# tzeitim/rogtk

Measured on AMD Instinct MI355X. Metric: reads/s UMI score+cluster, 150 bp/12 bp UMI, 1→8 MI355X; % HBM roofline, higher is better.
Workload: dtype u32/f64

## Files before the change

rogtk_amd/csrc/cluster_kernels.hip:

```cpp
#include <hip/hip_ext.h>
#include <hipcub/hipcub.hpp>

#include <algorithm>
#include <cstdlib>
#include <map>
#include <mutex>

#include <atomic>
#include <thread>
#include <chrono>
#include <cstring>

#include "rogtk_internal.h"

namespace rogtk {
namespace {

constexpr int kBlock = 256;
constexpr int kMarkParts = 8;
constexpr int kMarkChunks = 256;
constexpr int kScanWords = 1024;
constexpr int kLocal8Words = 1024;
constexpr int kLocal8Cap = 8192;
constexpr int kLocal8BigCap = 16384;
constexpr int kMaxRounds = 64;
constexpr int kRoundBatch = 4;

enum StatSlot { S_NDISTINCT = 0, S_NCLUSTERS = 1, S_OVERFLOW = 2, S_REDO = 3, S_ROUNDS = 4, S_P0 = 6,
                S_LCAP = 7 };
constexpr int kFlagsOff = 64;
constexpr int kStatsBytes = kFlagsOff + 4 * kMaxRounds;

__device__ __forceinline__ uint64_t rt_word(const uint4 e) { return (uint64_t)e.x | ((uint64_t)e.y << 32); }

__device__ __forceinline__ uint32_t rt_rank(const uint4 e, uint32_t code) {
    return e.z + (uint32_t)__popcll(rt_word(e) & ((1ull << (code & 63)) - 1ull));
}


__global__ __launch_bounds__(kBlock) void k_bitmap_wide(uint8_t* __restrict__ pres, int64_t words,
                                                        uint64_t* __restrict__ out) {
    const int64_t lane_g = (int64_t)blockIdx.x * kBlock + threadIdx.x;
    const int64_t w = lane_g >> 2;
    uint32_t m16 = 0;
    if (w < words) {
        uint4* p = reinterpret_cast<uint4*>(pres) + lane_g;
        const uint4 v = *p;
        const uint32_t x[4] = {v.x, v.y, v.z, v.w};
#pragma unroll
        for (int q = 0; q < 4; ++q) {
            const uint32_t b = x[q] & 0x01010101u;
            m16 |= ((b | (b >> 7) | (b >> 14) | (b >> 21)) & 0xFu) << (4 * q);
        }
        if (v.x | v.y | v.z | v.w) *p = make_uint4(0, 0, 0, 0);
    }
    uint64_t word = (uint64_t)m16 << (16 * (threadIdx.x & 3));
    word |= __shfl_xor(word, 1);
    word |= __shfl_xor(word, 2);
    if ((threadIdx.x & 3) == 0 && w < words) out[w] = word;
}

__global__ void k_bitmap_small(uint8_t* __restrict__ pres, uint64_t nbits, uint64_t* __restrict__ out) {
    if (threadIdx.x != 0 || blockIdx.x != 0) return;
    uint64_t m = 0;
    for (uint64_t b = 0; b < nbits; ++b) {
        if (pres[b]) m |= 1ull << b;
        pres[b] = 0;
    }
    out[0] = m;
}

template <int NT = kBlock>
__device__ __forceinline__ uint32_t block_excl_scan(uint32_t v, uint32_t* s_wave, uint32_t& total) {
    const int lane = threadIdx.x & 63, wave = threadIdx.x >> 6;
    uint32_t incl = v;
#pragma unroll
    for (int off = 1; off < 64; off <<= 1) {
        const uint32_t t = __shfl_up(incl, off);
        if (lane >= off) incl += t;
    }
    if (lane == 63) s_wave[wave] = incl;
    __syncthreads();
    uint32_t before = 0;
    total = 0;
#pragma unroll
    for (int k = 0; k < NT / 64; ++k) {
        const uint32_t s = s_wave[k];
        if (k < wave) before += s;
        total += s;
    }
    __syncthreads();
    return before + incl - v;
}

__global__ __launch_bounds__(kBlock) void k_scan_words(const uint64_t* __restrict__ bitmaps,
                                                       int n_bitmaps, int64_t words,
                                                       const unsigned long long* __restrict__ count_dev,
                                                       uint64_t* __restrict__ G,
                                                       uint32_t* __restrict__ wpref,
                                                       uint32_t* __restrict__ blksum) {
    __shared__ uint32_t s_wave[kBlock / 64];
    int64_t live = words;
    if (count_dev) live = min<int64_t>(words, (int64_t)((*count_dev + 63) / 64));
    const int64_t w0 = (int64_t)blockIdx.x * kScanWords + 4 * threadIdx.x;
    uint32_t c[4];
    uint32_t tsum = 0;
    uint64_t v[4] = {0, 0, 0, 0};
    for (int r = 0; r < n_bitmaps; ++r) {
        const uint64_t* b = bitmaps + (int64_t)r * words;
#pragma unroll
        for (int k = 0; k < 4; ++k)
// ... 962 lines not shown
                        if ((adj[a] >> b) & 1u) mn = root[b] < mn ? root[b] : mn;
                    x[0] = root[a];
                    x[1] = mn;
                    crossed |= CHECK ? x[0] != x[1] : hook_roots(T, f, x, 2, last_x, last_mn);
                }
            } else {
                uint64_t mm = multi;
                while (mm) {
                    const int b = __ffsll((long long)mm) - 1;
                    mm &= mm - 1;
                    const uint64_t below = (1ull << b) - 1ull;
                    int k = 0;
#pragma unroll
                    for (int v = 0; v < 4; ++v)
                        if ((m[v] >> b) & 1ull)
                            x[k++] = root[v] != kNone ? root[v]
                                                      : f[e[v].z + (uint32_t)__popcll(m[v] & below)];
                    if (CHECK) {
                        for (int v = 1; v < k; ++v) crossed |= x[v] != x[0];
                    } else {
                        crossed |= hook_roots(T, f, x, k, last_x, last_mn);
                    }
                }
            }
        }
    }
    const uint64_t crossed_bits = __ballot(crossed);
    if ((threadIdx.x & 63) == 0) {
        if (!CHECK && (u >> 6) < active_words) next[u >> 6] = crossed_bits;
        if (crossed_bits) flags[round] = 1u;
    }
    if (CHECK) return;
    __syncthreads();
    for (int k = threadIdx.x; k < kHookSlots; k += kBlock) {
        const uint32_t x = T.key[k];
        if (x == kNone) continue;
        if (T.val[k] < f[x]) atomicMin(f + x, T.val[k]);
    }
}

__global__ __launch_bounds__(kBlock) void k_hook_g(const uint4* __restrict__ RT, const uint32_t* __restrict__ UR,
                                                   int64_t words, int L, int p0, uint32_t* f,
                                                   unsigned int* __restrict__ flags, int round,
                                                   uint64_t* __restrict__ active, int64_t active_words,
                                                   const unsigned long long* __restrict__ stats) {
    hook_block<false>(blockIdx.x, RT, UR, words, L, p0, f, flags, round, active, active_words, stats);
}

__device__ __forceinline__ int64_t live_distinct(const unsigned long long* stats, int64_t max_distinct) {
    return min<int64_t>((int64_t)stats[S_NDISTINCT], max_distinct);
}

__global__ __launch_bounds__(kBlock) void k_jump(uint32_t* f, const uint64_t* __restrict__ lroot,
                                                 int64_t max_distinct,
                                                 const unsigned long long* __restrict__ stats,
                                                 const unsigned int* __restrict__ flags, int round) {
    if (flags[round] == 0 || stats[S_REDO]) return;
    const int64_t nd = live_distinct(stats, max_distinct);
    const int lane = threadIdx.x & 63;
    const int64_t nwaves = (int64_t)gridDim.x * (kBlock / 64);
    for (int64_t w = ((int64_t)blockIdx.x * kBlock + threadIdx.x) >> 6; w * 64 < nd; w += nwaves) {
        const uint64_t lr = lroot[w];
        const int64_t i = w * 64 + lane;
        if (!((lr >> lane) & 1ull) || i >= nd) continue;
        uint32_t r = f[i];
        if (r == (uint32_t)i) continue;
        for (uint32_t p = f[r]; p != r; p = f[r]) r = p;
        f[i] = r;
    }
}

constexpr int kRootWords = 64;

__device__ __forceinline__ void publish_stats(const unsigned long long* stats, unsigned long long* host,
                                              unsigned long long epoch) {
    for (int k = threadIdx.x; k < kStatsBytes / 8; k += blockDim.x)
        __hip_atomic_store(host + k, stats[k], __ATOMIC_RELAXED, __HIP_MEMORY_SCOPE_SYSTEM);
    __syncthreads();
    if (threadIdx.x == 0) {
        __hip_atomic_store(host + kStatsBytes / 8, epoch, __ATOMIC_RELEASE, __HIP_MEMORY_SCOPE_SYSTEM);
    }
}

__device__ __forceinline__ void roots_block(const int64_t bid, const uint32_t* __restrict__ f,
                                            const uint64_t* __restrict__ lroot, int64_t max_distinct,
                                            int64_t rwords, uint64_t* __restrict__ rbits,
                                            uint32_t* __restrict__ rpref, uint32_t* rblksum,
                                            const unsigned long long* stats) {
    __shared__ uint32_t s_cnt[kRootWords];
    const int64_t nd = live_distinct(stats, max_distinct);
    const int lane = threadIdx.x & 63, wave = threadIdx.x >> 6;
    constexpr int kPerWave = kRootWords / (kBlock / 64);
    const int64_t w0 = bid * kRootWords + wave * kPerWave;
    uint32_t fv[kPerWave];
    uint64_t lr[kPerWave];
#pragma unroll
    for (int k = 0; k < kPerWave; ++k) {
        const int64_t i = (w0 + k) * 64 + lane;
        lr[k] = (w0 + k) * 64 < nd ? lroot[w0 + k] : 0ull;
        fv[k] = i < nd ? f[i] : 0u;
    }
    uint64_t mine = 0;
#pragma unroll
    for (int k = 0; k < kPerWave; ++k) {
        const int64_t i = (w0 + k) * 64 + lane;
        const uint64_t m = __ballot(i < nd && ((lr[k] >> lane) & 1ull) && fv[k] == (uint32_t)i);
        if (lane == k) mine = m;
    }
    if (lane < kPerWave) {
        const int64_t w = w0 + lane;
        if (w < rwords) rbits[w] = mine;
        s_cnt[wave * kPerWave + lane] = (uint32_t)__popcll(mine);
    }
    __syncthreads();
    if (wave == 0) {
        const uint32_t v = lane < kRootWords ? s_cnt[lane] : 0u;
        uint32_t incl = v;
#pragma unroll
        for (int off = 1; off < 64; off <<= 1) {
            const uint32_t t = __shfl_up(incl, off);
            if (lane >= off) incl += t;
        }
        const int64_t w = bid * kRootWords + lane;
        if (lane < kRootWords && w < rwords) rpref[w] = incl - v;
        if (lane == kRootWords - 1) rblksum[bid] = incl;
    }
}

__global__ __launch_bounds__(kBlock) void k_roots_scan(const uint32_t* __restrict__ f,
                                                       const uint64_t* __restrict__ lroot, int64_t max_distinct,
                                                       int64_t rwords, uint64_t* __restrict__ rbits,
                                                       uint32_t* __restrict__ rpref, uint32_t* rblksum,
                                                       const unsigned long long* stats, unsigned long long* host,
                                                       unsigned long long epoch) {
    if (host && blockIdx.x == 0) publish_stats(stats, host, epoch);
    roots_block(blockIdx.x, f, lroot, max_distinct, rwords, rbits, rpref, rblksum, stats);
}

__global__ __launch_bounds__(kBlock) void k_roots_check(const uint32_t* __restrict__ f,
                                                        const uint64_t* __restrict__ lroot, int64_t max_distinct,
                                                        int64_t rwords, uint64_t* __restrict__ rbits,
                                                        uint32_t* __restrict__ rpref, uint32_t* rblksum,
                                                        const unsigned long long* stats, int64_t rblocks,
                                                        const uint4* __restrict__ RT, const uint32_t* __restrict__ UR,
                                                        int64_t words, int L, int p0, unsigned int* flags, int round,
                                                        uint64_t* active, int64_t active_words) {
    if ((int64_t)blockIdx.x < rblocks)
        roots_block(blockIdx.x, f, lroot, max_distinct, rwords, rbits, rpref, rblksum, stats);
    else
        hook_block<true>((int64_t)blockIdx.x - rblocks, RT, UR, words, L, p0, const_cast<uint32_t*>(f), flags,
                                round, active, active_words, stats);
}

__device__ __forceinline__ uint32_t root_label(uint32_t r, const uint64_t* __restrict__ rbits,
                                               const uint32_t* __restrict__ rpref,
                                               const uint32_t* __restrict__ rblkoff) {
    const uint32_t w = r >> 6;
    return rblkoff[w / kRootWords] + rpref[w] + (uint32_t)__popcll(rbits[w] & ((1ull << (r & 63)) - 1ull));
}

__device__ __forceinline__ void put_label(uint64_t c, uint32_t i, uint32_t lab, uint32_t* __restrict__ labelcode,
                                          uint32_t* __restrict__ ilab) {
    if (labelcode) labelcode[c] = lab;
    else ilab[i] = lab;
}

__global__ __launch_bounds__(kBlock) void k_word_label(const uint32_t* __restrict__ f,
                                                       const uint32_t* __restrict__ UR, int64_t words,
                                                       const uint4* __restrict__ RT, int64_t max_distinct,
                                                       const uint64_t* __restrict__ rbits,
                                                       const uint32_t* __restrict__ rpref,
                                                       const uint32_t* __restrict__ rblkoff,
                                                       uint32_t* __restrict__ wlab, uint64_t* __restrict__ wexc,
                                                       uint32_t* __restrict__ labelcode, uint32_t* __restrict__ ilab,
                                                       int exc1_on,
                                                       const uint32_t* __restrict__ rblksum = nullptr,
                                                       int64_t nrb_max = 0, unsigned long long* stats = nullptr,
                                                       const unsigned long long* pstats = nullptr,
                                                       unsigned long long* host = nullptr,
                                                       unsigned long long epoch = 0) {
    extern __shared__ uint32_t s_roff[];
    __shared__ uint32_t s_wave[kBlock / 64];
    if (host && blockIdx.x == 0) publish_stats(pstats, host, epoch);
    if (pstats[S_REDO]) return;
    if (rblksum) {
        const int64_t nd = live_distinct(stats, max_distinct);
        const int64_t nrb = min<int64_t>(nrb_max, (nd + (int64_t)kRootWords * 64 - 1) / ((int64_t)kRootWords * 64));
        uint32_t carry = 0;
        for (int64_t b0 = 0; b0 < nrb; b0 += kBlock) {
            const int64_t b = b0 + threadIdx.x;
            const uint32_t v = b < nrb ? rblksum[b] : 0u;
            uint32_t total;
            const uint32_t ex = block_excl_scan(v, s_wave, total);
            if (b < nrb) s_roff[b] = carry + ex;
            carry += total;
        }
        if (threadIdx.x == 0) {
            s_roff[nrb] = carry;
            if (blockIdx.x == 0) stats[S_NCLUSTERS] = carry;
        }
        __syncthreads();
        rblkoff = s_roff;
    }
    for (int64_t w = (int64_t)blockIdx.x * kBlock + threadIdx.x; w < words; w += (int64_t)gridDim.x * kBlock) {
        const uint32_t ur = UR[w];
        uint32_t root = kNone;
        uint64_t exc = 0;
        uint4 e = make_uint4(0, 0, 0, 0);
        uint64_t m = 0;
        if (ur != kNone) {
            root = f[ur];
        } else {
            e = RT[w];
            m = rt_word(e);
            const int cnt = __popcll(m);
            if (cnt > 0 && (int64_t)e.z + cnt <= max_distinct) {
                uint32_t cand = f[e.z], votes = 1;
                for (int k = 1; k < cnt; ++k) {
                    const uint32_t r = f[e.z + k];
                    if (r == cand) ++votes;
                    else if (votes == 0) {
                        cand = r;
                        votes = 1;
                    } else {
                        --votes;
                    }
                }
                root = cand;
                uint64_t mm = m;
                for (int k = 0; mm; ++k) {
                    const int b = __ffsll((long long)mm) - 1;
                    mm &= mm - 1;
                    if (f[e.z + k] != cand) exc |= 1ull << b;
                }
            }
        }
        uint32_t lab = root != kNone ? root_label(root, rbits, rpref, rblkoff) : kNone;
        if (exc && lab != kNone) {
            const uint64_t rest = exc & (exc - 1);
            if (exc1_on && !rest && lab < (1u << 24)) {
                lab |= 0xC0000000u | ((uint32_t)(__ffsll((long long)exc) - 1) << 24);
            } else if (exc1_on && !(rest & (rest - 1)) && lab < (1u << 17)) {
                lab |= 0xA0000000u | ((uint32_t)(__ffsll((long long)exc) - 1) << 17) |
                       ((uint32_t)(__ffsll((long long)rest) - 1) << 23);
            } else {
                lab = lab < 0x20000000u ? (lab | 0x80000000u) : kNone;
            }
        }
        wlab[w] = lab;
        uint64_t per_code = lab == kNone ? m : exc;
        while (per_code) {
            const int b = __ffsll((long long)per_code) - 1;
            per_code &= per_code - 1;
            const uint32_t i = e.z + (uint32_t)__popcll(m & ((1ull << b) - 1ull));
            if ((int64_t)i >= max_distinct) continue;
            const uint32_t li = root_label(f[i], rbits, rpref, rblkoff);
            put_label((uint64_t)w * 64 + b, i, li, labelcode, ilab);
        }
        wexc[w] = exc;
    }
}

__device__ __forceinline__ uint32_t word_label_of(const uint32_t* __restrict__ wlab,
                                                  const uint64_t* __restrict__ wexc, uint64_t c) {
    return decode_word_label(wlab[c >> 6], wexc, c);
}

template <int MODE, int G>
__global__ __launch_bounds__(kBlock) void k_assign(const uint32_t* __restrict__ codes,
                                                   const uint64_t* __restrict__ regbits, int64_t n,
                                                   const uint32_t* __restrict__ labelcode,
                                                   const uint32_t* __restrict__ flab,
                                                   const uint4* __restrict__ RT, const uint32_t* __restrict__ wlab,
                                                   const uint64_t* __restrict__ wexc, uint32_t* __restrict__ out) {
    constexpr int64_t kTile = 256 * G;
    const int lane = threadIdx.x & 63;
    const int64_t nwaves = (int64_t)gridDim.x * (kBlock / 64);
    for (int64_t tile = (((int64_t)blockIdx.x * kBlock + threadIdx.x) >> 6) * kTile; tile < n;
         tile += nwaves * kTile) {
        uint32_t c[G][4];
        uint32_t reg[G];
#pragma unroll
        for (int g = 0; g < G; ++g) {
            const int64_t row0 = tile + 256 * g + 4 * lane;
            c[g][0] = c[g][1] = c[g][2] = c[g][3] = 0;
            if (row0 + 4 <= n) {
                const u32x4_t v = stream_load(reinterpret_cast<const u32x4_t*>(codes + row0));
                c[g][0] = v.x; c[g][1] = v.y; c[g][2] = v.z; c[g][3] = v.w;
            } else {
                for (int k = 0; k < 4; ++k)
                    if (row0 + k < n) c[g][k] = codes[row0 + k];
            }
            reg[g] = row0 >= n ? 0u : regbits ? (uint32_t)(regbits[row0 >> 6] >> (row0 & 63)) & 0xFu : 0xFu;
        }
        uint32_t id[G][4];
#pragma unroll
        for (int g = 0; g < G; ++g)
#pragma unroll
            for (int k = 0; k < 4; ++k) {
                id[g][k] = 0xFFFFFFFFu;
                if ((reg[g] >> k) & 1u) {
                    const uint32_t wl = wlab ? word_label_of(wlab, wexc, c[g][k]) : kNone;
                    id[g][k] = wl != kNone ? wl
                               : MODE == 0 ? labelcode[c[g][k]]
                               : MODE == 1 ? flab[rt_rank(RT[c[g][k] >> 6], c[g][k])]
                                           : rt_rank(RT[c[g][k] >> 6], c[g][k]);
                }
            }
#pragma unroll
        for (int g = 0; g < G; ++g) {
            const int64_t row0 = tile + 256 * g + 4 * lane;
            if (row0 + 4 <= n) {
                stream_store(u32x4_t{id[g][0], id[g][1], id[g][2], id[g][3]}, reinterpret_cast<u32x4_t*>(out + row0));
            } else {
                for (int k = 0; k < 4; ++k)
                    if (row0 + k < n) out[row0 + k] = id[g][k];
            }
        }
    }
}

template <int MODE>
__global__ __launch_bounds__(kBlock) void k_lookup(const uint64_t* __restrict__ q, int64_t nq, uint64_t nbits,
                                                   const uint32_t* __restrict__ labelcode,
                                                   const uint32_t* __restrict__ flab, const uint4* __restrict__ RT,
                                                   const uint32_t* __restrict__ wlab,
                                                   const uint64_t* __restrict__ wexc, uint32_t* __restrict__ out) {
    for (int64_t i = (int64_t)blockIdx.x * kBlock + threadIdx.x; i < nq; i += (int64_t)gridDim.x * kBlock) {
        const uint64_t c = q[i];
        uint32_t lab = kNone;
        if (c < nbits) {
            const uint4 e = RT[c >> 6];
            if ((rt_word(e) >> (c & 63)) & 1ull) {
                const uint32_t wl = wlab ? word_label_of(wlab, wexc, c) : kNone;
                lab = wl != kNone ? wl : MODE == 0 ? labelcode[c] : flab[rt_rank(e, (uint32_t)c)];
            }
        }
        out[i] = lab;
    }
}

inline int grid_for(int64_t lanes, int64_t cap = 0) {
    int64_t g = (lanes + kBlock - 1) / kBlock;
    if (g < 1) g = 1;
    if (cap && g > cap) g = cap;
    return (int)g;
}

struct WsPtrs {
    unsigned long long* stats;
    unsigned int* flags;
    uint8_t* presence;
    uint64_t* G;
    uint4* RT;
    uint32_t *wpref, *blksum, *blkoff, *D, *f, *UR;
    uint64_t *rbits, *lroot;
    uint32_t *rpref, *rblksum, *rblkoff, *labelcode, *ilab;
    uint64_t* active;
    uint64_t* lb;
};

inline WsPtrs ws_ptrs(const ClusterLayout& cl, uint8_t* ws) {
    WsPtrs p;
    p.stats = (unsigned long long*)(ws + cl.off_stats);
    p.flags = (unsigned int*)(ws + cl.off_stats + kFlagsOff);
    p.presence = ws + cl.off_presence;
    p.G = (uint64_t*)(ws + cl.off_bitmap);
    p.RT = (uint4*)(ws + cl.off_rt);
    p.wpref = (uint32_t*)(ws + cl.off_wpref);
    p.blksum = (uint32_t*)(ws + cl.off_blksum);
    p.blkoff = (uint32_t*)(ws + cl.off_blkoff);
    p.D = (uint32_t*)(ws + cl.off_D);
    p.f = (uint32_t*)(ws + cl.off_f);
    p.UR = (uint32_t*)(ws + cl.off_ur);
    p.rbits = (uint64_t*)(ws + cl.off_rbits);
    p.lroot = (uint64_t*)(ws + cl.off_lroot);
    p.rpref = (uint32_t*)(ws + cl.off_rpref);
    p.rblksum = (uint32_t*)(ws + cl.off_rblksum);
    p.rblkoff = (uint32_t*)(ws + cl.off_rblkoff);
    p.labelcode = cl.label_by_code ? (uint32_t*)(ws + cl.off_labelcode) : nullptr;
    p.ilab = cl.label_by_code ? nullptr : (uint32_t*)(ws + cl.off_ilab);
    p.active = (uint64_t*)(ws + cl.off_active);
    p.lb = (uint64_t*)(ws + cl.off_lb);
    return p;
}

constexpr int64_t kPersistentGrid = 2048;

}

int cluster_layout(int L, int64_t max_distinct, ClusterLayout* o) {
    ROGTK_REQUIRE(L >= 1 && L <= kMaxPackedLen, ROGTK_E_UNSUPPORTED,
                  "cluster: umi_len %d outside 1..%d", L, kMaxPackedLen);
    ROGTK_REQUIRE(max_distinct >= 1 && max_distinct <= 0xFFFFFFFFll, ROGTK_E_INVALID,
                  "cluster: max_distinct %lld outside 1..2^32-1", (long long)max_distinct);
    ClusterLayout c{};
    c.L = L;
    c.nbits = 1ull << (2 * L);
    if ((uint64_t)max_distinct > c.nbits) max_distinct = (int64_t)c.nbits;
    c.max_distinct = max_distinct;
    c.words = (int64_t)((c.nbits + 63) / 64);
    c.blocks = (c.words + kScanWords - 1) / kScanWords;
    c.rwords = (max_distinct + 63) / 64;
    c.rblocks = (c.rwords + kRootWords - 1) / kRootWords;
    c.label_by_code = L <= 13;
    int64_t off = 0;
    auto take = [&](int64_t bytes) {
        const int64_t at = off;
        off += (bytes + 255) / 256 * 256;
        return at;
    };
    c.off_stats = take(kStatsBytes);
    c.off_presence = take((int64_t)(c.nbits < 64 ? 64 : c.nbits));
    c.off_bitmap = take(c.words * 8);
    c.off_rt = take(c.words * 16);
    c.off_wpref = take(c.words * 4);
    c.off_blksum = take(c.blocks * 4);
    c.off_blkoff = take((c.blocks + 1) * 4);
    c.off_D = take(max_distinct * 4);
    c.off_f = take(max_distinct * 4);
    c.off_ur = take(c.words * 4);
    c.off_rbits = take(c.rwords * 8);
    c.off_lroot = take(c.rwords * 8);
    c.off_rpref = take(c.rwords * 4);
    c.off_rblksum = take(c.rblocks * 4);
    c.off_rblkoff = take((c.rblocks + 1) * 4);
    c.off_labelcode = c.label_by_code ? take((int64_t)c.nbits * 4) : off;
    c.off_ilab = c.label_by_code ? off : take(max_distinct * 4);
    const int64_t tasks = L > kLocalPos ? (int64_t)(L - kLocalPos) * (c.words >> 2) : 0;
    c.active_words = (tasks + 63) / 64;
    c.off_active = take(2 * std::max<int64_t>(c.active_words, 1) * 8);
    c.off_lb = take((2 * std::max(c.blocks, c.rblocks) + 1) * 8);
    c.total = off;
    *o = c;
    return ROGTK_OK;
}


__global__ __launch_bounds__(kBlock) void k_mark_xcd(const uint32_t* __restrict__ codes,
                                                      const uint64_t* __restrict__ regbits, int64_t n,
                                                      int two_l, int64_t chunk, uint8_t* __restrict__ pres) {
    const uint32_t part = blockIdx.x % kMarkParts;
    const int64_t c0 = (int64_t)(blockIdx.x / kMarkParts) * chunk;
    const int64_t c1 = c0 + chunk < n ? c0 + chunk : n;
    for (int64_t r = c0 + 4 * (int64_t)threadIdx.x; r < c1; r += 4 * kBlock) {
        uint32_t c[4];
        uint32_t reg = regbits ? (uint32_t)(regbits[r >> 6] >> (r & 63)) & 0xFu : 0xFu;
        if (r + 4 <= n) {
            const u32x4_t v = stream_load(reinterpret_cast<const u32x4_t*>(codes + r));
            c[0] = v.x; c[1] = v.y; c[2] = v.z; c[3] = v.w;
        } else {
            reg &= (1u << (uint32_t)(n - r)) - 1u;
            for (int k = 0; k < 4; ++k) c[k] = r + k < n ? codes[r + k] : 0u;
        }
#pragma unroll
        for (int k = 0; k < 4; ++k)
            if (((reg >> k) & 1u) && (uint32_t)(((uint64_t)c[k] * kMarkParts) >> two_l) == part)
                pres[c[k]] = 1;
    }
}

int launch_cluster_mark(const uint32_t* codes, const uint64_t* regular_bits, int64_t n, int L,
                        uint8_t* presence, hipStream_t s) {
    if (n <= 0) return ROGTK_OK;
    ProfScope prof(K_MARK, s);
    int64_t chunk = (n + kMarkChunks - 1) / kMarkChunks;
    chunk = (chunk + 4 * kBlock - 1) / (4 * kBlock) * (4 * kBlock);
    const int64_t chunks = (n + chunk - 1) / chunk;
    hipLaunchKernelGGL(k_mark_xcd, dim3((unsigned)(chunks * kMarkParts)), dim3(kBlock), 0, s, codes, regular_bits,
                       n, 2 * L, chunk, presence);
    ROGTK_HIP_CHECK(hipGetLastError());
    return ROGTK_OK;
}

int launch_cluster_local_bitmap(const ClusterLayout& cl, uint8_t* ws, uint64_t* out, hipStream_t s) {
    WsPtrs p = ws_ptrs(cl, ws);
    ProfScope prof(K_BITMAP, s);
    if (cl.nbits >= 64) {
        hipLaunchKernelGGL(k_bitmap_wide, dim3(grid_for(cl.words * 4)), dim3(kBlock), 0, s, p.presence,
                           cl.words, out);
    } else {
        hipLaunchKernelGGL(k_bitmap_small, dim3(1), dim3(64), 0, s, p.presence, cl.nbits, out);
    }
    ROGTK_HIP_CHECK(hipGetLastError());
    return ROGTK_OK;
}

namespace {

constexpr int kSpecRounds = 4;
std::atomic<int> g_spec_rounds{kSpecRounds};
std::atomic<bool> g_spec_adaptive{true};
std::atomic<int> g_lb_polls{kLbMaxPolls};

struct ResolveState {
    uint8_t* hstats = nullptr;
    uint8_t* hstats_dev = nullptr;
    uint64_t epoch = 0;
    int launched = 0;
    bool pending = false;
    int rounds = 0;
    int needed = 0;
    bool word_labels = false;
    bool exact = false;
    uint32_t scan_tag = 0;
    int lcc_choice = -1;
    bool checked = false;
    ClusterLayout cl{};
    struct {
        bool on = false;
        const uint32_t* codes;
        const uint64_t* regbits;
        int64_t n;
        uint32_t* cid;
    } deferred;
};
std::mutex g_rs_mu;
std::map<const void*, ResolveState> g_rs;

int wait_published(const ResolveState& st) {
    const volatile unsigned long long* seq = (const volatile unsigned long long*)(st.hstats + kStatsBytes);
    const auto t0 = std::chrono::steady_clock::now();
    while (*seq != st.epoch) {
        std::this_thread::yield();
        ROGTK_REQUIRE(std::chrono::steady_clock::now() - t0 < std::chrono::seconds(120), ROGTK_E_HIP,
                      "cluster: resolve flags not published within 120 s (stream stalled?)");
    }
    std::atomic_thread_fence(std::memory_order_acquire);
    return ROGTK_OK;
}

int enqueue_rounds(const ClusterLayout& cl, const WsPtrs& p, int from, int to, hipStream_t s) {
    const int pg = grid_for(cl.max_distinct, kPersistentGrid);
    const int64_t tasks = (int64_t)(cl.L - kLocalPos) * (cl.words >> 2);
    for (int k = from; k < to; ++k) {
        ROGTK_TIMED_LAUNCH(K_K_HOOK, k_hook_g, dim3(grid_for(tasks)), dim3(kBlock), 0, s, p.RT, p.UR, cl.words, cl.L, kLocalPos,
                           p.f, p.flags, k, p.active, cl.active_words, (const unsigned long long*)p.stats);
        ROGTK_TIMED_LAUNCH(K_K_JUMP, k_jump, dim3(pg), dim3(kBlock), 0, s, p.f, p.lroot, cl.max_distinct, p.stats, p.flags, k);
    }
    ROGTK_HIP_CHECK(hipGetLastError());
    return ROGTK_OK;
}

thread_local hipEvent_t t_resolve_fin = nullptr;

int enqueue_labels(const ClusterLayout& cl, const WsPtrs& p, hipStream_t s,
                   unsigned long long* host_stats = nullptr, int check_round = -1, uint64_t epoch = 0) {
    const bool lds_off = (cl.rblocks + 1) * 4 <= 65536;
    {
        ProfScope prof(K_FLATTEN, s);
        if (check_round >= 0) {
            const int64_t tasks = (int64_t)(cl.L - kLocalPos) * (cl.words >> 2);
            ROGTK_TIMED_LAUNCH(K_K_ROOTS, k_roots_check, dim3((unsigned)(cl.rblocks + grid_for(tasks))), dim3(kBlock), 0, s, p.f,
                               p.lroot, cl.max_distinct, cl.rwords, p.rbits, p.rpref, p.rblksum,
                               (const unsigned long long*)p.stats, cl.rblocks, p.RT, p.UR, cl.words, cl.L, kLocalPos,
                               p.flags, check_round, p.active, cl.active_words);
        } else {
            ROGTK_TIMED_LAUNCH(K_K_ROOTS, k_roots_scan, dim3((unsigned)cl.rblocks), dim3(kBlock), 0, s, p.f, p.lroot,
                               cl.max_distinct, cl.rwords, p.rbits, p.rpref, p.rblksum,
                               (const unsigned long long*)p.stats, host_stats, (unsigned long long)epoch);
        }
        if (!lds_off)
            hipLaunchKernelGGL(k_scan_blocks, dim3(1), dim3(kBlock), 0, s, p.rblksum, cl.rblocks, p.rblkoff, p.stats,
                               (int)S_NCLUSTERS, -1, 0, (int64_t)kRootWords * 64);
        ROGTK_HIP_CHECK(hipGetLastError());
    }
    {
        ProfScope prof(K_LABEL, s);
        static const int exc1_on = [] {
            const char* e = getenv("ROGTK_WORD_EXC1");
            return e && e[0] == '0' ? 0 : 1;
        }();
        if (t_resolve_fin) arm_attached_event(t_resolve_fin);
        ROGTK_TIMED_LAUNCH(K_K_WORD_LABEL, k_word_label, dim3(grid_for(cl.words, kPersistentGrid)), dim3(kBlock),
                           lds_off ? (size_t)(cl.rblocks + 1) * 4 : 0, s, p.f, p.UR, cl.words, p.RT, cl.max_distinct,
                           p.rbits, p.rpref, p.rblkoff, p.wpref, p.G, p.labelcode, p.ilab, exc1_on,
                           lds_off ? p.rblksum : nullptr, (int64_t)cl.rblocks, lds_off ? p.stats : nullptr,
                           (const unsigned long long*)p.stats, check_round >= 0 ? host_stats : nullptr,
                           (unsigned long long)epoch);
        if (t_resolve_fin && attached_event_taken()) t_resolve_fin = nullptr;
        ROGTK_HIP_CHECK(hipGetLastError());
    }
    return ROGTK_OK;
}

int first_zero(const unsigned int* f, int from, int to) {
    for (int k = from; k < to; ++k)
        if (f[k] == 0) return k;
    return -1;
}

}

#ifndef ROGTK_ASSIGN_WGS
#define ROGTK_ASSIGN_WGS 2
#endif
#ifndef ROGTK_ASSIGN_G
#define ROGTK_ASSIGN_G 2
#endif
namespace {
int enqueue_assign(const ClusterLayout& cl, const WsPtrs& p, int labels, const uint32_t* codes,
                   const uint64_t* regular_bits, int64_t n, uint32_t* cluster_id, hipStream_t s);
int finish_locked(const void* ws, ResolveState& st, hipStream_t s, int* redone = nullptr);
}

namespace {
bool fused_scan_enabled() {
    static const bool on = [] {
        const char* e = getenv("ROGTK_FUSED_SCAN");
        return !(e && e[0] == '0');
    }();
    return on;
}

bool lcc_predict_enabled() {
    static const bool on = [] {
        const char* e = getenv("ROGTK_LCC_PREDICT");
        return !(e && e[0] == '0');
    }();
    return on;
}

int enqueue_resolve(const ClusterLayout& cl, const WsPtrs& p, const uint64_t* bitmaps, int n_bitmaps,
                    int max_distance, int spec, unsigned long long* host_stats, uint64_t epoch, hipStream_t s,
                    uint32_t scan_tag, int lcc_choice, bool* checked) {
    *checked = false;
    {
        ProfScope prof(K_SCAN, s);
        if (scan_tag) {
            ROGTK_TIMED_LAUNCH(K_K_SCAN_RT, k_scan_rt, dim3((unsigned)cl.blocks), dim3(kBlock), 0, s, bitmaps, n_bitmaps, cl.words,
                               p.RT, p.lroot, max_distance == 0 ? (int64_t)0 : cl.rwords,
                               p.lb + std::max(cl.blocks, cl.rblocks) + 1, p.lb, scan_tag, p.stats, (int)S_NDISTINCT,
                               max_distance == 0 ? (int)S_NCLUSTERS : -1, local8_enabled() ? cl.L : 0,
                               local8_big_enabled(), g_lb_polls.load());
        } else {
            hipLaunchKernelGGL(k_scan_words, dim3((unsigned)cl.blocks), dim3(kBlock), 0, s, bitmaps, n_bitmaps,
                               cl.words, (const unsigned long long*)nullptr, p.G, p.wpref, p.blksum);
            hipLaunchKernelGGL(k_scan_blocks, dim3(1), dim3(kBlock), 0, s, p.blksum, cl.blocks, p.blkoff, p.stats,
                               (int)S_NDISTINCT, max_distance == 0 ? (int)S_NCLUSTERS : -1, 1, (int64_t)0,
                               local8_enabled() ? cl.L : 0, local8_big_enabled());
            hipLaunchKernelGGL(k_rt, dim3(grid_for(cl.words)), dim3(kBlock), 0, s, p.G, cl.words, p.wpref, p.blkoff,
                               p.RT, p.lroot, max_distance == 0 ? 0 : cl.rwords);
        }
    }
    if (max_distance == 0) {
        const int cgrid = grid_for((int64_t)std::min<uint64_t>(cl.nbits, 1ull << 30), 16384);
        hipLaunchKernelGGL(k_build_d, dim3(cgrid), dim3(kBlock), 0, s, p.RT, cl.nbits, p.D, p.f, p.labelcode, p.ilab,
                           cl.max_distinct, p.stats);
        return hipGetLastError() == hipSuccess ? 0 : -1;
    }
    ProfScope prof(K_UNION, s);
    launch_local_cc(p.RT, cl.words, cl.L, p.f, p.UR, p.lroot, cl.rwords, cl.max_distinct, p.stats, s, lcc_choice);
    if (cl.L <= kLocalPos) {
        if (enqueue_labels(cl, p, s, nullptr)) return -1;
        return hipGetLastError() == hipSuccess ? 0 : -1;
    }
    const bool fuse = host_stats && spec >= 2;
    const int real = fuse ? spec - 1 : spec;
    if (enqueue_rounds(cl, p, 0, real, s)) return -1;
    *checked = fuse;
    if (enqueue_labels(cl, p, s, host_stats, fuse ? real : -1, epoch)) return -1;
    return hipGetLastError() == hipSuccess ? real : -1;
// ... 175 lines not shown
    return enqueue_assign(cl, p, wl, codes, regular_bits, n, cluster_id, s);
}

int cluster_assign_prepare(const ClusterLayout& cl, const uint8_t* ws, const uint32_t* codes,
                           const uint64_t* regular_bits, int64_t n, uint32_t* cluster_id, hipStream_t s,
                           bool deferred, AssignIn* a) {
    a->wlab = nullptr;
    a->wexc = nullptr;
    a->labelcode = nullptr;
    a->out = nullptr;
    if (!deferred)
        if (int rc = cluster_finish(ws, s)) return rc;
    bool wl = false;
    {
        std::lock_guard<std::mutex> lk(g_rs_mu);
        auto it = g_rs.find(ws);
        if (it != g_rs.end()) {
            wl = it->second.word_labels;
            if (deferred && it->second.pending) {
                auto& d = it->second.deferred;
                d.on = true;
                d.codes = codes;
                d.regbits = regular_bits;
                d.n = n;
                d.cid = cluster_id;
            }
        }
    }
    if (!wl || !cl.label_by_code) return ROGTK_OK;
    WsPtrs p = ws_ptrs(cl, const_cast<uint8_t*>(ws));
    a->wlab = p.wpref;
    a->wexc = p.G;
    a->labelcode = p.labelcode;
    a->out = cluster_id;
    return ROGTK_OK;
}

int launch_cluster_lookup(const ClusterLayout& cl, const uint8_t* ws, const uint64_t* q, int64_t nq, uint32_t* lab,
                          hipStream_t s) {
    if (nq <= 0) return ROGTK_OK;
    if (int rc = cluster_finish(ws, s)) return rc;
    WsPtrs p = ws_ptrs(cl, const_cast<uint8_t*>(ws));
    bool wl = false;
    {
        std::lock_guard<std::mutex> lk(g_rs_mu);
        auto it = g_rs.find(ws);
        if (it != g_rs.end()) wl = it->second.word_labels;
    }
    const uint32_t* wlab = wl ? p.wpref : nullptr;
    const uint64_t* wexc = wl ? p.G : nullptr;
    const int g = grid_for(nq, 4096);
    if (cl.label_by_code)
        hipLaunchKernelGGL(k_lookup<0>, dim3(g), dim3(kBlock), 0, s, q, nq, cl.nbits, p.labelcode, p.D, p.RT, wlab,
                           wexc, lab);
    else
        hipLaunchKernelGGL(k_lookup<1>, dim3(g), dim3(kBlock), 0, s, q, nq, cl.nbits, p.labelcode, p.ilab, p.RT, wlab,
                           wexc, lab);
    ROGTK_HIP_CHECK(hipGetLastError());
    return ROGTK_OK;
}

#ifndef ROGTK_ASSIGN_WGS
#define ROGTK_ASSIGN_WGS 2
#endif
#ifndef ROGTK_ASSIGN_G
#define ROGTK_ASSIGN_G 2
#endif
namespace {
int enqueue_assign(const ClusterLayout& cl, const WsPtrs& p, int labels, const uint32_t* codes,
                   const uint64_t* regular_bits, int64_t n, uint32_t* cluster_id, hipStream_t s) {
    if (n <= 0) return ROGTK_OK;
    const uint32_t* wlab = labels == 1 ? p.wpref : nullptr;
    const uint64_t* wexc = labels == 1 ? p.G : nullptr;
    ProfScope prof(K_ASSIGN, s, true);
    static const int64_t cap = [] {
        int dev = 0, cus = 0;
        if (hipGetDevice(&dev) != hipSuccess ||
            hipDeviceGetAttribute(&cus, hipDeviceAttributeMultiprocessorCount, dev) != hipSuccess || cus <= 0)
            cus = 256;
        return (int64_t)ROGTK_ASSIGN_WGS * cus;
    }();
    constexpr int kGroups = ROGTK_ASSIGN_G;
    const int g = grid_for((n + 4 * kGroups - 1) / (4 * kGroups), cap);
    if (labels == 2)
        hipExtLaunchKernelGGL((k_assign<2, kGroups>), dim3(g), dim3(kBlock), 0, s, prof.start(), prof.stop(), 0, codes,
                              regular_bits, n, p.labelcode, p.ilab, p.RT, wlab, wexc, cluster_id);
    else if (cl.label_by_code)
        hipExtLaunchKernelGGL((k_assign<0, kGroups>), dim3(g), dim3(kBlock), 0, s, prof.start(), prof.stop(), 0, codes,
                              regular_bits, n, p.labelcode, p.D, p.RT, wlab, wexc, cluster_id);
    else
        hipExtLaunchKernelGGL((k_assign<1, kGroups>), dim3(g), dim3(kBlock), 0, s, prof.start(), prof.stop(), 0, codes,
                              regular_bits, n, p.labelcode, p.ilab, p.RT, wlab, wexc, cluster_id);
    ROGTK_HIP_CHECK(hipGetLastError());
    return ROGTK_OK;
}
}



namespace {

constexpr int kPartBits = 8;
constexpr int kPartBlock = 512;

__global__ __launch_bounds__(kBlock) void k_mark_keys(const uint32_t* __restrict__ codes,
                                                      const uint64_t* __restrict__ regbits, int64_t n,
                                                      uint32_t* __restrict__ keys) {
    const int64_t i = (int64_t)blockIdx.x * kBlock + threadIdx.x;
    if (i >= n) return;
    const bool reg = (regbits[i >> 6] >> (i & 63)) & 1ull;
    keys[i] = reg ? codes[i] : 0xFFFFFFFFu;
}

__device__ int64_t wg_lower_bound(const uint32_t* __restrict__ a, int64_t n, uint64_t v) {
    int64_t lo = 0, hi = n;
    while (lo < hi) {
        const int64_t step = (hi - lo + kPartBlock - 1) / kPartBlock;
        const int64_t pos = lo + (int64_t)threadIdx.x * step;
        const bool less = pos < hi && (uint64_t)a[pos] < v;
        const int64_t cnt = __syncthreads_count(less);
        const int64_t nlo = cnt ? lo + (cnt - 1) * step + 1 : lo;
        const int64_t nhi = min(hi, lo + cnt * step);
        lo = nlo;
        hi = nhi;
    }
    return lo;
}

__global__ __launch_bounds__(kPartBlock) void k_part_bitmap(const uint32_t* __restrict__ sorted, int64_t n,
                                                            int two_l, uint64_t* __restrict__ bitmap) {
    extern __shared__ uint32_t lbits[];
    const int p = blockIdx.x;
    const int shift = two_l - kPartBits;
    const uint32_t pwords32 = (1u << shift) >> 5;
    for (uint32_t k = threadIdx.x; k < pwords32; k += kPartBlock) lbits[k] = 0;
    __shared__ int64_t range[2];
    const int64_t r0 = wg_lower_bound(sorted, n, (uint64_t)p << shift);
    const int64_t r1 = p + 1 == (1 << kPartBits) ? n : wg_lower_bound(sorted, n, (uint64_t)(p + 1) << shift);
    if (threadIdx.x == 0) {
        range[0] = r0;
        range[1] = r1;
    }
    __syncthreads();
    const uint32_t mask = (1u << shift) - 1u;
    constexpr int kUnroll = 8;
    const int64_t rend = range[1];
    for (int64_t i0 = range[0] + threadIdx.x; i0 < rend; i0 += (int64_t)kPartBlock * kUnroll) {
        uint32_t key[kUnroll];
#pragma unroll
        for (int u = 0; u < kUnroll; ++u) {
            const int64_t i = i0 + (int64_t)u * kPartBlock;
            key[u] = i < rend ? __builtin_nontemporal_load(sorted + i) : 0xFFFFFFFFu;
        }
#pragma unroll
        for (int u = 0; u < kUnroll; ++u) {
            if ((uint64_t)key[u] >> two_l) continue;
            const uint32_t c = key[u] & mask;
            atomicOr(&lbits[c >> 5], 1u << (c & 31));
        }
    }
    __syncthreads();
    uint64_t* out = bitmap + ((uint64_t)p << shift >> 6);
    for (uint32_t k = threadIdx.x; k < pwords32 / 2; k += kPartBlock)
        out[k] = (uint64_t)lbits[2 * k] | ((uint64_t)lbits[2 * k + 1] << 32);
}

#ifndef ROGTK_SLICE_BLOCK
#define ROGTK_SLICE_BLOCK 1024
#endif
constexpr int kSliceBlock = ROGTK_SLICE_BLOCK;
constexpr int kSliceChunks = 8;
#ifndef ROGTK_SLICE_LOG2
#define ROGTK_SLICE_LOG2 20
#endif
constexpr int kSliceLog2 = ROGTK_SLICE_LOG2;
// ... 333 lines not shown
```

rogtk_amd/csrc/rogtk_internal.h:

```cpp
#pragma once

#include <hip/hip_runtime.h>

#include <algorithm>
#include <cstddef>
#include <cstdint>
#include <functional>
#include <vector>

#include "../../include/rogtk_hip.h"

namespace rogtk {

void set_error(const char* fmt, ...) __attribute__((format(printf, 1, 2)));
int require_device();

#define ROGTK_HIP_CHECK(expr)                                                                    \
    do {                                                                                         \
        hipError_t e_ = (expr);                                                                  \
        if (e_ != hipSuccess) {                                                                  \
            ::rogtk::set_error("%s failed: %s (%s:%d)", #expr, hipGetErrorString(e_), __FILE__, \
                               __LINE__);                                                        \
            return ROGTK_E_HIP;                                                                  \
        }                                                                                        \
// ... 121 lines not shown
    if ((wl >> 29) & 1u)
        return b != ((wl >> 17) & 63u) && b != ((wl >> 23) & 63u) ? (wl & 0x1FFFFu) : 0xFFFFFFFFu;
    return ((wexc[c >> 6] >> b) & 1ull) ? 0xFFFFFFFFu : (wl & 0x1FFFFFFFu);
}

#ifndef ROGTK_NT_SCORE_STORE
#define ROGTK_NT_SCORE_STORE 1
#endif
template <class V>
__device__ __forceinline__ void score_store(V v, V* p) {
#if ROGTK_NT_SCORE_STORE
    stream_store(v, p);
#else
    *p = v;
#endif
}

struct PackedParams {
    double sh[kMaxPackedLen + 1];
    double di[kMaxPackedLen + 1];
    double ling[kMaxPackedLen + 1];
    double frac[kMaxPackedLen + 1];
    int L;
    int ham_mode;
    uint32_t tcode, cmplo, always_mismatch, max_distance;
};

struct ScoreOut {
    double* sh;
    double* ling;
    double* homo;
    double* di;
    uint32_t* longest;
    double* dust;
    double* comb;
};

inline ScoreOut to_score_out(const rogtk_umi_scores* s) {
    if (!s) return ScoreOut{nullptr, nullptr, nullptr, nullptr, nullptr, nullptr, nullptr};
    return ScoreOut{s->shannon_entropy,      s->linguistic_complexity, s->homopolymer_fraction,
                    s->dinucleotide_entropy, s->longest_homopolymer_run, s->dust_score,
                    s->combined_score};
}
inline bool any_score(const ScoreOut& o) {
    return o.sh || o.ling || o.homo || o.di || o.longest || o.dust || o.comb;
}

void encode_target(const uint8_t* target, int64_t target_len, int L, uint32_t max_distance,
                   PackedParams* p);
int build_packed_params(int L, PackedParams* p);

struct AssignIn {
    const uint32_t* wlab;
    const uint64_t* wexc;
    const uint32_t* labelcode;
    uint32_t* out;
};

int launch_stage(const void* offsets, int offset_width, const uint8_t* values,
                 const uint8_t* validity, int64_t validity_offset, int64_t n, int L,
                 uint32_t* codes, uint64_t* regular_bits, int64_t* irregular_rows,
                 unsigned long long* n_irregular, hipStream_t s);
int launch_score_packed(const uint32_t* codes, const uint64_t* regular_bits, int64_t n,
                        const PackedParams& p, const ScoreOut& o, uint32_t* hd, uint64_t* hw, hipStream_t s,
                        const AssignIn* asg = nullptr);
int launch_score_rows(const void* offsets, int offset_width, const uint8_t* values,
                      const int64_t* rows, const int64_t* n_rows_dev, int64_t max_rows,
                      const double* lut, int64_t lut_max, const ScoreOut& o,
                      const uint8_t* target_dev, int64_t target_len, int ham, uint32_t max_distance,
                      uint32_t* hd, uint64_t* hw, hipStream_t s);

struct ClusterLayout {
    int L;
    int64_t max_distinct;
    uint64_t nbits;
    int64_t words;
    int64_t blocks;
    int64_t rwords;
    int64_t rblocks;
    bool label_by_code;
    int64_t off_stats, off_presence, off_bitmap, off_rt, off_wpref, off_blksum, off_blkoff, off_D, off_f, off_ur,
        off_rbits, off_lroot, off_rpref, off_rblksum, off_rblkoff, off_labelcode, off_ilab, off_active,
        active_words, off_lb, total;
};
int cluster_layout(int L, int64_t max_distinct, ClusterLayout* out);

struct DevBuf {
    void* p = nullptr;
    size_t cap = 0;
    std::vector<void*> retired;
    ~DevBuf() {
        if (p) hipFree(p);
        for (void* q : retired) hipFree(q);
    }
    int ensure(size_t bytes) {
        if (bytes <= cap && p) return ROGTK_OK;
        size_t grow = 0;
        if (p) {
            retired.push_back(p);
            p = nullptr;
            grow = cap + cap / 2;
            cap = 0;
        }
        size_t want = std::max<size_t>(std::max(bytes, grow), 256);
        want = (want + 255) / 256 * 256;
        ROGTK_HIP_CHECK(hipMalloc(&p, want));
        cap = want;
        return ROGTK_OK;
    }
    void reclaim() {
        for (void* q : retired) hipFree(q);
        retired.clear();
    }
    template <class T>
    T* as() const { return reinterpret_cast<T*>(p); }
};


int launch_cluster_mark(const uint32_t* codes, const uint64_t* regular_bits, int64_t n, int L,
                        uint8_t* presence, hipStream_t s);
int launch_cluster_local_bitmap(const ClusterLayout& cl, uint8_t* ws, uint64_t* bitmap_out,
                                hipStream_t s);
int cluster_mark_bitmap_temp(int64_t n, int L, int64_t* bytes);
int launch_cluster_mark_bitmap(const uint32_t* codes, const uint64_t* regular_bits, int64_t n, int L,
                               uint64_t* bitmap, void* temp, int64_t temp_bytes, hipStream_t s);
int launch_cluster_mark_phase(const uint32_t* codes, const uint64_t* regular_bits, int64_t n, int L,
                              uint64_t* bitmap, void* temp, int64_t temp_bytes, int phase, hipStream_t s);
int cluster_assign_prepare(const ClusterLayout& cl, const uint8_t* ws, const uint32_t* codes,
                           const uint64_t* regular_bits, int64_t n, uint32_t* cluster_id, hipStream_t s,
                           bool deferred, AssignIn* a);
int launch_cluster_resolve(const ClusterLayout& cl, uint8_t* ws, const uint64_t* bitmaps,
                           int n_bitmaps, int max_distance, hipStream_t s);
int cluster_finish(const void* ws, hipStream_t s, int* redone = nullptr);
void cluster_release(const void* ws);
int cluster_rounds(const void* ws, hipStream_t s, int* rounds);
int cluster_set_spec_rounds(int n);
int cluster_set_lookback_polls(int n);
int cluster_set_mark_method(int m);
int launch_cluster_assign(const ClusterLayout& cl, const uint8_t* ws, const uint32_t* codes,
                          const uint64_t* regular_bits, int64_t n, uint32_t* cluster_id,
                          hipStream_t s, bool deferred = false);

int irregular_cluster(const void* offsets, int offset_width, const uint8_t* values,
                      const int64_t* rows, int64_t n_rows, int64_t max_len, const int64_t* stats_dev,
                      uint32_t* cluster_id, int64_t* n_irregular_clusters, hipStream_t s);

using CodeLookup = std::function<int(const uint64_t* q, int64_t nq, uint32_t* lab, hipStream_t s)>;
int irregular_merge(const void* offsets, int offset_width, const uint8_t* values, const int64_t* rows,
                    int64_t n_rows, int64_t max_len, int L, int64_t n_reg, const CodeLookup* lookup,
                    uint32_t* relabel, int64_t relabel_n, uint32_t* cluster_id, int64_t* n_clusters, hipStream_t s);
int sorted_code_lookup(const uint64_t* G, int64_t ng, const uint32_t* labels, const uint64_t* q, int64_t nq,
                       uint32_t* lab, hipStream_t s);
int launch_cluster_lookup(const ClusterLayout& cl, const uint8_t* ws, const uint64_t* q, int64_t nq, uint32_t* lab,
                          hipStream_t s);

int masked_records_range(const uint64_t* D, int64_t nd, int p0, int np, uint64_t* mk, uint32_t* pos, uint64_t* code,
                         hipStream_t s);

int cc_labels(int64_t nv, const uint32_t* edges, int64_t m, uint32_t* labels, int64_t* n_clusters, hipStream_t s);

struct SortedCodes;
struct DevCol;
using ExtraCodeBytes = std::function<int(int64_t m, size_t* bytes)>;
int sorted_distinct_codes(const DevCol& col, int L, bool want_counts, const ExtraCodeBytes* extra, uint32_t* cluster_id,
                          SortedCodes* out, hipStream_t s, const uint32_t* groups = nullptr);

// ... 60 lines not shown
```

Baseline: 38.38 billion.

## Fast-path dominant cluster label in assign via sampled root and LDS bitmap

Samples 256 words in the roots kernel to find a dominant cluster root and stores it in the stats slot. The word-label kernel then writes a per-word bitmap of codes belonging to that root, and the assign kernel loads this bitmap into LDS. Codes found in it take the dominant label directly, skipping the word-label and label-table lookups. This adds sampling work, an extra bitmap write, and LDS use per block that grows with the number of words, which is why it is enabled only for L up to 12.

```diff
diff --git a/rogtk_amd/csrc/cluster_kernels.hip b/rogtk_amd/csrc/cluster_kernels.hip
--- a/rogtk_amd/csrc/cluster_kernels.hip
+++ b/rogtk_amd/csrc/cluster_kernels.hip
@@ -26,7 +26,7 @@
 constexpr int kMaxRounds = 64;
 constexpr int kRoundBatch = 4;
 
-enum StatSlot { S_NDISTINCT = 0, S_NCLUSTERS = 1, S_OVERFLOW = 2, S_REDO = 3, S_ROUNDS = 4, S_P0 = 6,
+enum StatSlot { S_NDISTINCT = 0, S_NCLUSTERS = 1, S_OVERFLOW = 2, S_REDO = 3, S_ROUNDS = 4, S_DOM = 5, S_P0 = 6,
                 S_LCAP = 7 };
 constexpr int kFlagsOff = 64;
 constexpr int kStatsBytes = kFlagsOff + 4 * kMaxRounds;
@@ -1155,6 +1155,47 @@
     }
 }
 
+constexpr int kDomSample = kBlock;
+constexpr int kDomHeader = 2;
+constexpr uint64_t kDomNoLabel = ~0ull;
+constexpr int kDomMaxL = 12;
+
+__device__ __forceinline__ void pick_dominant(const uint32_t* __restrict__ f, const uint32_t* __restrict__ UR,
+                                              const uint4* __restrict__ RT, int64_t words, int64_t max_distinct,
+                                              unsigned long long* dom) {
+    __shared__ uint32_t s_samp[kDomSample];
+    __shared__ unsigned long long s_best[kBlock / 64];
+    const int64_t ns = min<int64_t>(kDomSample, words);
+    const int64_t w = (int64_t)threadIdx.x * (words / ns);
+    uint32_t r = kNone;
+    if ((int64_t)threadIdx.x < ns) {
+        uint32_t i = UR[w];
+        if (i == kNone) {
+            const uint4 e = RT[w];
+            if (rt_word(e)) i = e.z;
+        }
+        if ((int64_t)i < max_distinct) r = f[i];
+    }
+    s_samp[threadIdx.x] = r;
+    __syncthreads();
+    uint32_t cnt = 0;
+    if (r != kNone)
+        for (int k = 0; k < kDomSample; ++k) cnt += s_samp[k] == r;
+    unsigned long long key = r != kNone ? ((unsigned long long)cnt << 32) | (0xFFFFFFFFu - r) : 0ull;
+#pragma unroll
+    for (int off = 32; off; off >>= 1) {
+        const unsigned long long o = __shfl_xor(key, off);
+        key = o > key ? o : key;
+    }
+    if ((threadIdx.x & 63) == 0) s_best[threadIdx.x >> 6] = key;
+    __syncthreads();
+    if (threadIdx.x == 0) {
+        for (int k = 1; k < kBlock / 64; ++k) key = s_best[k] > key ? s_best[k] : key;
+        const bool any = (int64_t)(key >> 32) * 4 >= ns && key != 0;
+        *dom = any ? (unsigned long long)(0xFFFFFFFFu - (uint32_t)key) + 1ull : 0ull;
+    }
+}
+
 __device__ __forceinline__ void roots_block(const int64_t bid, const uint32_t* __restrict__ f,
                                             const uint64_t* __restrict__ lroot, int64_t max_distinct,
                                             int64_t rwords, uint64_t* __restrict__ rbits,
@@ -1205,8 +1246,12 @@
                                                        int64_t rwords, uint64_t* __restrict__ rbits,
                                                        uint32_t* __restrict__ rpref, uint32_t* rblksum,
                                                        const unsigned long long* stats, unsigned long long* host,
-                                                       unsigned long long epoch) {
+                                                       unsigned long long epoch, int64_t rblocks,
+                                                       const uint4* __restrict__ RT, const uint32_t* __restrict__ UR,
+                                                       int64_t words) {
     if (host && blockIdx.x == 0) publish_stats(stats, host, epoch);
+    if ((int64_t)blockIdx.x == (rblocks > 1 ? 1 : 0))
+        pick_dominant(f, UR, RT, words, max_distinct, const_cast<unsigned long long*>(stats) + S_DOM);
     roots_block(blockIdx.x, f, lroot, max_distinct, rwords, rbits, rpref, rblksum, stats);
 }
 
@@ -1218,9 +1263,11 @@
                                                         const uint4* __restrict__ RT, const uint32_t* __restrict__ UR,
                                                         int64_t words, int L, int p0, unsigned int* flags, int round,
                                                         uint64_t* active, int64_t active_words) {
-    if ((int64_t)blockIdx.x < rblocks)
+    if ((int64_t)blockIdx.x < rblocks) {
+        if ((int64_t)blockIdx.x == (rblocks > 1 ? 1 : 0))
+            pick_dominant(f, UR, RT, words, max_distinct, const_cast<unsigned long long*>(stats) + S_DOM);
         roots_block(blockIdx.x, f, lroot, max_distinct, rwords, rbits, rpref, rblksum, stats);
-    else
+    } else
         hook_block<true>((int64_t)blockIdx.x - rblocks, RT, UR, words, L, p0, const_cast<uint32_t*>(f), flags,
                                 round, active, active_words, stats);
 }
@@ -1251,7 +1298,8 @@
                                                        int64_t nrb_max = 0, unsigned long long* stats = nullptr,
                                                        const unsigned long long* pstats = nullptr,
                                                        unsigned long long* host = nullptr,
-                                                       unsigned long long epoch = 0) {
+                                                       unsigned long long epoch = 0,
+                                                       uint64_t* __restrict__ wdom = nullptr) {
     extern __shared__ uint32_t s_roff[];
     __shared__ uint32_t s_wave[kBlock / 64];
     if (host && blockIdx.x == 0) publish_stats(pstats, host, epoch);
@@ -1275,6 +1323,9 @@
         __syncthreads();
         rblkoff = s_roff;
     }
+    const uint32_t dom = wdom ? (uint32_t)pstats[S_DOM] - 1u : kNone;
+    if (wdom && blockIdx.x == 0 && threadIdx.x == 0)
+        wdom[0] = dom != kNone ? (uint64_t)root_label(dom, rbits, rpref, rblkoff) : kDomNoLabel;
     for (int64_t w = (int64_t)blockIdx.x * kBlock + threadIdx.x; w < words; w += (int64_t)gridDim.x * kBlock) {
         const uint32_t ur = UR[w];
         uint32_t root = kNone;
@@ -1321,6 +1372,10 @@
             }
         }
         wlab[w] = lab;
+        if (wdom) {
+            const uint64_t b = __ballot(lab != kNone && root == dom && !exc);
+            if ((threadIdx.x & 63) == 0) wdom[kDomHeader + (w >> 6)] = b;
+        }
         uint64_t per_code = lab == kNone ? m : exc;
         while (per_code) {
             const int b = __ffsll((long long)per_code) - 1;
@@ -1339,13 +1394,31 @@
     return decode_word_label(wlab[c >> 6], wexc, c);
 }
 
-template <int MODE, int G>
+template <int MODE, int G, bool DOM = false>
 __global__ __launch_bounds__(kBlock) void k_assign(const uint32_t* __restrict__ codes,
                                                    const uint64_t* __restrict__ regbits, int64_t n,
                                                    const uint32_t* __restrict__ labelcode,
                                                    const uint32_t* __restrict__ flab,
                                                    const uint4* __restrict__ RT, const uint32_t* __restrict__ wlab,
-                                                   const uint64_t* __restrict__ wexc, uint32_t* __restrict__ out) {
+                                                   const uint64_t* __restrict__ wexc, uint32_t* __restrict__ out,
+                                                   const uint64_t* __restrict__ wdom, int dom_words) {
+    extern __shared__ __attribute__((aligned(16))) uint32_t s_dom[];
+    uint32_t dom_label = 0;
+    bool dom_on = false;
+    if (DOM) {
+        const uint64_t h = wdom[0];
+        dom_on = h != kDomNoLabel;
+        dom_label = (uint32_t)h;
+        if (dom_on) {
+            if (dom_words >= 2) {
+                const uint4* src = reinterpret_cast<const uint4*>(wdom + kDomHeader);
+                for (int i = threadIdx.x; i < dom_words / 2; i += kBlock) reinterpret_cast<uint4*>(s_dom)[i] = src[i];
+            } else if (threadIdx.x < 2) {
+                s_dom[threadIdx.x] = reinterpret_cast<const uint32_t*>(wdom + kDomHeader)[threadIdx.x];
+            }
+            __syncthreads();
+        }
+    }
     constexpr int64_t kTile = 256 * G;
     const int lane = threadIdx.x & 63;
     const int64_t nwaves = (int64_t)gridDim.x * (kBlock / 64);
@@ -1373,6 +1446,10 @@
             for (int k = 0; k < 4; ++k) {
                 id[g][k] = 0xFFFFFFFFu;
                 if ((reg[g] >> k) & 1u) {
+                    if (DOM && dom_on && ((s_dom[c[g][k] >> 11] >> ((c[g][k] >> 6) & 31u)) & 1u)) {
+                        id[g][k] = dom_label;
+                        continue;
+                    }
                     const uint32_t wl = wlab ? word_label_of(wlab, wexc, c[g][k]) : kNone;
                     id[g][k] = wl != kNone ? wl
                                : MODE == 0 ? labelcode[c[g][k]]
@@ -1431,6 +1508,7 @@
     uint32_t *rpref, *rblksum, *rblkoff, *labelcode, *ilab;
     uint64_t* active;
     uint64_t* lb;
+    uint64_t* wdom;
 };
 
 inline WsPtrs ws_ptrs(const ClusterLayout& cl, uint8_t* ws) {
@@ -1455,6 +1533,7 @@
     p.ilab = cl.label_by_code ? nullptr : (uint32_t*)(ws + cl.off_ilab);
     p.active = (uint64_t*)(ws + cl.off_active);
     p.lb = (uint64_t*)(ws + cl.off_lb);
+    p.wdom = cl.dom_words ? (uint64_t*)(ws + cl.off_wdom) : nullptr;
     return p;
 }
 
@@ -1504,6 +1583,8 @@
     c.active_words = (tasks + 63) / 64;
     c.off_active = take(2 * std::max<int64_t>(c.active_words, 1) * 8);
     c.off_lb = take((2 * std::max(c.blocks, c.rblocks) + 1) * 8);
+    c.dom_words = L <= kDomMaxL ? (c.words + 63) / 64 : 0;
+    c.off_wdom = take(c.dom_words ? (kDomHeader + c.dom_words + 1) * 8 : 0);
     c.total = off;
     *o = c;
     return ROGTK_OK;
@@ -1631,7 +1712,8 @@
         } else {
             ROGTK_TIMED_LAUNCH(K_K_ROOTS, k_roots_scan, dim3((unsigned)cl.rblocks), dim3(kBlock), 0, s, p.f, p.lroot,
                                cl.max_distinct, cl.rwords, p.rbits, p.rpref, p.rblksum,
-                               (const unsigned long long*)p.stats, host_stats, (unsigned long long)epoch);
+                               (const unsigned long long*)p.stats, host_stats, (unsigned long long)epoch, cl.rblocks,
+                               p.RT, p.UR, cl.words);
         }
         if (!lds_off)
             hipLaunchKernelGGL(k_scan_blocks, dim3(1), dim3(kBlock), 0, s, p.rblksum, cl.rblocks, p.rblkoff, p.stats,
@@ -1650,7 +1732,7 @@
                            p.rbits, p.rpref, p.rblkoff, p.wpref, p.G, p.labelcode, p.ilab, exc1_on,
                            lds_off ? p.rblksum : nullptr, (int64_t)cl.rblocks, lds_off ? p.stats : nullptr,
                            (const unsigned long long*)p.stats, check_round >= 0 ? host_stats : nullptr,
-                           (unsigned long long)epoch);
+                           (unsigned long long)epoch, p.wdom);
         if (t_resolve_fin && attached_event_taken()) t_resolve_fin = nullptr;
         ROGTK_HIP_CHECK(hipGetLastError());
     }
@@ -1992,15 +2074,27 @@
     }();
     constexpr int kGroups = ROGTK_ASSIGN_G;
     const int g = grid_for((n + 4 * kGroups - 1) / (4 * kGroups), cap);
-    if (labels == 2)
+    static const bool dom_on = [] {
+        const char* e = getenv("ROGTK_ASSIGN_DOM");
+        return !(e && e[0] == '0');
+    }();
+    if (labels == 1 && cl.label_by_code && p.wdom && dom_on) {
+        const int dw = (int)cl.dom_words;
+        hipExtLaunchKernelGGL((k_assign<0, kGroups, true>), dim3(g), dim3(kBlock), (size_t)(dw + (dw & 1)) * 8, s,
+                              prof.start(), prof.stop(), 0, codes, regular_bits, n, p.labelcode, p.D, p.RT, wlab, wexc,
+                              cluster_id, (const uint64_t*)p.wdom, dw);
+    } else if (labels == 2)
         hipExtLaunchKernelGGL((k_assign<2, kGroups>), dim3(g), dim3(kBlock), 0, s, prof.start(), prof.stop(), 0, codes,
-                              regular_bits, n, p.labelcode, p.ilab, p.RT, wlab, wexc, cluster_id);
+                              regular_bits, n, p.labelcode, p.ilab, p.RT, wlab, wexc, cluster_id,
+                              (const uint64_t*)nullptr, 0);
     else if (cl.label_by_code)
         hipExtLaunchKernelGGL((k_assign<0, kGroups>), dim3(g), dim3(kBlock), 0, s, prof.start(), prof.stop(), 0, codes,
-                              regular_bits, n, p.labelcode, p.D, p.RT, wlab, wexc, cluster_id);
+                              regular_bits, n, p.labelcode, p.D, p.RT, wlab, wexc, cluster_id,
+                              (const uint64_t*)nullptr, 0);
     else
         hipExtLaunchKernelGGL((k_assign<1, kGroups>), dim3(g), dim3(kBlock), 0, s, prof.start(), prof.stop(), 0, codes,
-                              regular_bits, n, p.labelcode, p.ilab, p.RT, wlab, wexc, cluster_id);
+                              regular_bits, n, p.labelcode, p.ilab, p.RT, wlab, wexc, cluster_id,
+                              (const uint64_t*)nullptr, 0);
     ROGTK_HIP_CHECK(hipGetLastError());
     return ROGTK_OK;
 }
diff --git a/rogtk_amd/csrc/rogtk_internal.h b/rogtk_amd/csrc/rogtk_internal.h
--- a/rogtk_amd/csrc/rogtk_internal.h
+++ b/rogtk_amd/csrc/rogtk_internal.h
@@ -227,6 +227,7 @@
     int64_t off_stats, off_presence, off_bitmap, off_rt, off_wpref, off_blksum, off_blkoff, off_D, off_f, off_ur,
         off_rbits, off_lroot, off_rpref, off_rblksum, off_rblkoff, off_labelcode, off_ilab, off_active,
         active_words, off_lb, total;
+    int64_t off_wdom, dom_words;
 };
 int cluster_layout(int L, int64_t max_distinct, ClusterLayout* out);
 
```

Measured after the change: 39.15 billion (median of 6 runs). 1.02x the previous value.
